# segasai/rvspecfit

Measured on AMD Instinct MI355X. Metric: spectra/sec (CCF+chi2 grid) DESI 3-arm, higher is better.
Workload: dtype f64

## Files before the change

### include/rvsgpu.h

```cpp
#ifndef RVSGPU_H
#define RVSGPU_H
#include <stdint.h>

#ifdef __cplusplus
extern "C" {
#endif

#define RVS_E_ARG (-1)
#define RVS_E_LAUNCH (-2)

#define RVS_ST_SPLINE_RANGE 0x1
#define RVS_ST_SPLINE_GRID 0x2
#define RVS_ST_NONFINITE 0x4
#define RVS_ST_CHOL_FALLBACK 0x8
#define RVS_ST_OUTSIDE_NAN 0x10
#define RVS_ST_CCF_FAILED 0x20
#define RVS_ST_ALLMASKED 0x40
#define RVS_ST_QUAD_ASSERT 0x80
#define RVS_ST_ILLCOND 0x100
#define RVS_ST_NONPOS_MEDIAN 0x200
#define RVS_ST_RBF_NOTPD 0x400

#define RVS_ABI_VERSION 18
int rvs_abi_version(void);
// ... 314 lines not shown
                     int32_t *status, void *stream);

int rvs_ccf_preprocess(const double *lam, const double *spec,
                       const double *espec, const uint8_t *badmask, int npix,
                       int B, int continuum, const double *Eb, const int32_t *El,
                       const double *Cinv, const int32_t *istart, int nnode,
                       const int32_t *bin_start, const int32_t *xind,
                       const double *rw, int nfft, double maxerr,
                       double *proc_spec, double *proc_ivar, double *sse,
                       double *cont, double *pfit, int32_t *status,
                       void *stream);
int rvs_ccf_preprocess_g(const double *lam, const double *spec, const double *espec,
                         const uint8_t *badmask, int npix, int B, int continuum,
                         const double *Eb, const int32_t *El, const double *Cinv,
                         const int32_t *istart, int nnode,
                         const int32_t *bin_start, const int32_t *xind,
                         const double *rw, int nfft, double maxerr,
                         double *proc_spec, double *proc_ivar, double *sse,
                         double *cont, double *pfit, int32_t *status,
                         const int32_t *grid_id, const int32_t *npix_g,
                         const int32_t *nnode_g, void *stream);

int rvs_ccf_fft_pos(int nfft, int f);
int rvs_ccf_xcorr(const double *proc_spec, const double *proc_ivar, int nfft,
                  int B, const double *tfft, const double *tfft2, int T,
                  const double *twid, int continuum, const int32_t *lag_pos,
                  const double *lag_vel, int nlag, const int32_t *ilo,
                  const double *vgrid, int nvel, double beta,
                  const uint8_t *prune, double *chisq, double *work,
                  void *stream);

#define RVS_CCF_MODEL_MAX_NTP 9216
int rvs_ccf_model_rows(const float *dats, int64_t ngrid, const int64_t *sel,
                       int exp_flag, int ntp, int M, double *rows, void *stream);
int rvs_ccf_models_build(const double *rows, const uint8_t *f32row,
                         const double *erows, int ntp, int M, int continuum,
                         const double *Eb, const int32_t *El, const double *Cinv,
                         const int32_t *istart, int nnode, const int32_t *bin_start,
                         const double *lnlam, const double *logl, const int32_t *ihi,
                         int npoints, const double *twid, double *model, double *fft,
                         double *fft2, double *cont, double *pfit, int32_t *status,
                         void *stream);

int rvs_ccf_select(const double *chisq, const double *sse, int narm_sse, int B,
                   int T, const double *vgrid, int nvel, double *res,
                   double *best_ccf, int32_t *status, void *stream);

int rvs_template_nn(const double *params, int B, int ndim, uint32_t log_mask,
                    const double *M, const double *S, int nlayer,
                    const float *const *W, const float *const *b,
                    const int32_t *dims, float *act0, float *act1,
                    double *templ, void *stream);

int rvs_template_nn_grad(const double *params, int B, int ndim, uint32_t log_mask,
                         const double *M, const double *S, int nlayer,
                         const float *const *W, const float *const *b,
                         const int32_t *dims, float *act0, float *act1,
                         double *templ , void *stream);

int rvs_nn_outside(const double *params, int B, int ndim, uint32_t log_mask,
                   const double *M, const double *S, int mapped,
                   const double *xeqs, int nfx, const double *yeqs, int nfy,
                   double *outside, void *stream);

int rvs_nm_begin(int S, int N, double xatol, double fatol, int maxiter,
                 const double *sim, const double *fsim, const int32_t *nit,
                 int32_t *flags, int32_t *list1, double *X1, int32_t *counts,
                 int jbound, void *stream);
int rvs_nm_decide(int N, const double *sim, const double *fsim,
// ... 293 lines not shown
```

### rvspecfit_amd/_lib.py

```python
import ctypes
import os

import torch

_HERE = os.path.dirname(os.path.abspath(__file__))
LIB_PATH = os.path.join(_HERE, 'librvsgpu.so')

P = ctypes.c_void_p
I = ctypes.c_int
L = ctypes.c_int64
D = ctypes.c_double
U = ctypes.c_uint32

SIGNATURES = {
    'rvs_abi_version': (I, []),
    'rvs_option_set': (I, [ctypes.c_char_p, I]),
    'rvs_option_get': (I, [ctypes.c_char_p, P]),
    'rvs_template_polylinear': (I, [P, L, I, P, P, P, I, P, P, U, I, P, I, P, P,
                                    P, P, P]),
    'rvs_template_polylinear_grad': (I, [P, L, I, P, P, P, I, P, P, U, I, P, I, P,
                                         P, P, P, P]),
    'rvs_template_tri': (I, [P, I, P, P, P, I, I, U, I, P, I, P, P, P, P, P]),
    'rvs_template_tri_buckets': (I, [P, I, P, P, P, I, I, U, I, P, P, I, P, P, P,
                                     P, P]),
# ... 91 lines not shown
    'rvs_objective_work_size': (L, [I, I]),
    'rvs_objective_fused': (I, [P, I, I, P, P, P, I, P, D, I, P, P, P, P]),
    'rvs_objective_from_template': (I, [P, I, I, P, P, P, P, I, P, D, I, P, P, P,
                                        P]),
    'rvs_objective_fused_n': (I, [P, I, I, P, P, P, I, P, P, D, I, P, P, P, P]),
    'rvs_objective_from_template_n': (I, [P, I, I, P, P, P, P, I, P, P, D, I, P,
                                          P, P, P]),
    'rvs_objective_grad_ok': (I, [I, I, I, I, I]),
    'rvs_objective_grad_work_size': (L, [I, I, I]),
    'rvs_objective_grad': (I, [P, I, I, I, P, P, P, I, P, D, P, P, P, P, P, P]),
    'rvs_bfgs_run_grad_fused': (I, [P, P, P, P, P, P, I, P, P]),
    'rvs_grid_moments': (I, [P, P, L, P, I, I, I, I, P, P, P, P]),
    'rvs_basis_build': (I, [P, P, I, I, I, I, P, P, P, P, P]),
    'rvs_ccf_tables_build': (I, [P, P, I, I, P, I, I, P, P, P, I, P, P, P, P, P, P,
                                 P]),
    'rvs_ccf_preprocess': (I, [P, P, P, P, I, I, I, P, P, P, P, I, P, P, P, I, D,
                               P, P, P, P, P, P, P]),
    'rvs_ccf_preprocess_g': (I, [P, P, P, P, I, I, I, P, P, P, P, I, P, P, P, I,
                                 D, P, P, P, P, P, P, P, P, P, P]),
    'rvs_ccf_fft_pos': (I, [I, I]),
    'rvs_ccf_xcorr': (I, [P, P, I, I, P, P, I, P, I, P, P, I, P, P, I, D, P, P,
                          P, P]),
    'rvs_ccf_select': (I, [P, P, I, I, I, P, I, P, P, P, P]),
    'rvs_ccf_model_rows': (I, [P, L, P, I, I, I, P, P]),
    'rvs_ccf_models_build': (I, [P, P, P, I, I, I, P, P, P, P, I, P, P, P, P, I, P,
                                 P, P, P, P, P, P, P]),
    'rvs_template_nn': (I, [P, I, I, U, P, P, I, P, P, P, P, P, P, P]),
    'rvs_template_nn_grad': (I, [P, I, I, U, P, P, I, P, P, P, P, P, P, P]),
    'rvs_template_nn_arms': (I, [P, I, I, I, P, P]),
    'rvs_template_nn_arms_n': (I, [P, I, P, I, I, P, P]),
    'rvs_nn_outside': (I, [P, I, I, U, P, P, I, P, I, P, I, P, P]),
    'rvs_rebin_weights': (I, [P, I, P, P, P, P, I, I, P, P]),
    'rvs_rebin_apply': (I, [P, I, L, I, I, P, P, I, P, P, P, I, I, P, P]),
    'rvs_template_normalize': (I, [P, I, I, P, I, D, D, I, I, P, P, P, P]),
    'rvs_rbf_work_size': (L, [I, I]),
    'rvs_rbf_factor': (I, [P, I, I, D, P, P, P, P]),
    'rvs_rbf_solve': (I, [P, I, L, I, I, P, P, P]),
    'rvs_rbf_eval': (I, [P, I, P, I, I, D, P, I, I, P, L, P]),
    'rvs_nn_train_work_size': (L, [I, I, I, P]),
    'rvs_nn_train_grad': (I, [P, P, I, P, I, I, P, P, P, P, P, D, P, P, P, P, P, P]),
    'rvs_nn_adam_step': (I, [I, P, P, P, P, P, P, P, P, P, D, I, P]),
    'rvs_nn_train_epoch': (I, [P, P, I, P, I, I, I, P, P, P, P, P, P, P, P, P, D, D, I,
                               P, P, P, P]),
}

_lib = None
# ... 216 lines not shown
```

### rvspecfit_amd/csrc/ccf.hip

```cpp
#include "common.h"

#define PP_NT 512
#define PP_LOG2NT 9
#define PP_NW (PP_NT / 64)


#define SEL_NB PP_NT
struct SelShared {
  unsigned long long kmin, kmax, result, next, cand[64];
  int hist[SEL_NB];
  int wtot[PP_NW];
  int cnt, nnan, nc, bucket, kk, nle;
};
__device__ __forceinline__ unsigned long long sel_key(double x) {
  const unsigned long long b = (unsigned long long)__double_as_longlong(x);
  return (b >> 63) ? ~b : (b | 0x8000000000000000ull);
}
__device__ __forceinline__ double sel_value(unsigned long long k) {
  const unsigned long long b = (k >> 63) ? (k & 0x7fffffffffffffffull) : ~k;
  return __longlong_as_double((long long)b);
}
__device__ __forceinline__ unsigned long long shfl_xor_u64(unsigned long long v,
                                                           int o) {
  const int lo = __shfl_xor((int)(v & 0xffffffffu), o, 64);
// ... 1020 lines not shown
    return RVS_E_ARG;
  if ((fft != nullptr) != (fft2 != nullptr)) return RVS_E_ARG;
  if (fft) {
    if (npoints < 64 || npoints > 16384 || (npoints & (npoints - 1)) || !twid)
      return RVS_E_ARG;
  }
  const size_t shm = sizeof(double) * 2 * (size_t)ntp;
  static bool attr_set = false;
  if (!attr_set) {
    (void)hipFuncSetAttribute(
        (const void *)ccf_model_kernel, hipFuncAttributeMaxDynamicSharedMemorySize,
        (int)(CCF_MODEL_LDS - sizeof(LMSharedModel) - sizeof(SelShared)));
    (void)hipGetLastError();
    attr_set = true;
  }
  hipLaunchKernelGGL(ccf_model_kernel, dim3(M), dim3(PP_NT), shm, rvs_stream(stream),
                     rows, f32row, erows, ntp, continuum, Eb, El, Cinv, istart, nnode,
                     bin_start, lnlam, logl, ihi, npoints, model, cont, pfit, status);
  RVS_LAUNCH_CHECK();
  if (fft) return ccf_model_rfft(model, npoints, M, twid, fft, fft2, rvs_stream(stream));
  return 0;
}

__device__ __forceinline__ bool nan_less(double a, long long ka, double b,
                                         long long kb) {
  const bool an = !(a == a), bn = !(b == b);
  if (an != bn) return an;
  if (an) return ka < kb;
  return (a < b) || (a == b && ka < kb);
}

__global__ void __launch_bounds__(256)
    ccf_select_kernel(const double *__restrict__ chisq,
                      const double *__restrict__ sse, int narm, int T,
                      const double *__restrict__ vgrid, int nvel,
                      double *__restrict__ res, double *__restrict__ best_ccf,
                      int32_t *__restrict__ status) {
  __shared__ double sv[4];
  __shared__ long long sk[4];
  const int b = blockIdx.x, tid = threadIdx.x;
  double tot = 0;
  for (int a = 0; a < narm; a++) tot += sse[(int64_t)a * gridDim.x + b];
  const double *c = chisq + (int64_t)b * T * nvel;
  double bv = __builtin_inf();
  long long bk = (1ll << 62);
  for (int e = tid; e < T * nvel; e += 256) {
    const double x = c[e] + tot;
    if (nan_less(x, e, bv, bk)) {
      bv = x;
      bk = e;
    }
  }
#pragma unroll
  for (int o = 32; o > 0; o >>= 1) {
// ... 64 lines not shown
```

### rvspecfit_amd/csrc/ccf_fft.hip

```cpp
#include "common.h"

#define XC_NT 512
#define XC_NTW(n2) ((n2) >> 3)

struct XcLds {
  int t1;
  int c0;
  int t1c;
  int ca;
  int lt;
  size_t bytes;
};
#define XW_NT1C 73
#define XW_NLT 256
#define XC_LDS_MAX (159 * 1024)
__host__ __device__ constexpr XcLds xc_lds_pair(int n2, int nlag) {
  const int t1 = n2, c0 = t1 + XC_NTW(n2);
  return {t1, c0, 0, 0, 0,
          sizeof(double2) * (size_t)c0 + sizeof(double) * 2 * (size_t)nlag};
}
__host__ __device__ constexpr XcLds xc_lds_ws(int n2, int nlag, bool ratio) {
  const int t1 = 2 * n2, c0 = t1 + XC_NTW(n2), t1c = c0 + ((nlag + 1) >> 1),
            ca = t1c + XW_NT1C, lt = ca + (ratio ? (nlag + 1) >> 1 : 0);
  return {t1, c0, t1c, ca, lt,
          sizeof(double2) * (size_t)lt + sizeof(int32_t) * (size_t)XW_NLT};
}
__host__ __device__ constexpr XcLds xc_lds_ws2(int n2, int nlag) {
  const int t1 = 4 * n2, c0 = t1 + XC_NTW(n2);
  return {t1, c0, 0, 0, 0,
          sizeof(double2) * (size_t)c0 + sizeof(double) * 2 * (size_t)nlag};
}
__host__ __device__ constexpr bool xc_lds_fits(const XcLds &L, int n2, int nimg,
                                               int nrow, int nlag, bool ws, bool ratio) {
  const size_t D2 = sizeof(double2), D = sizeof(double);
  size_t end = D2 * (size_t)nimg * n2;
  if (D2 * L.t1 < end) return false;
  end = D2 * (L.t1 + XC_NTW(n2));
  if (D2 * L.c0 < end) return false;
  end = D2 * L.c0 + D * (size_t)nrow * nlag;
  if (ws) {
    if (D2 * L.t1c < end) return false;
    end = D2 * (L.t1c + 72);
    if (D2 * L.ca < end) return false;
    end = D2 * L.ca + (ratio ? D * (size_t)nlag : 0);
    if (D2 * L.lt < end) return false;
    end = D2 * L.lt + sizeof(int32_t) * (size_t)XW_NLT;
  }
  return end <= L.bytes && L.bytes <= XC_LDS_MAX;
}
constexpr bool xc_lds_check() {
  for (int nlag = 2; nlag <= 512; nlag++)
    for (int n2 = 2048; n2 <= 4096; n2 *= 2) {
      for (int ratio = 0; ratio < 2; ratio++)
        if (!xc_lds_fits(xc_lds_ws(n2, nlag, ratio), n2, 2, 1, nlag, true, ratio))
          return false;
      if (n2 == 2048 && !xc_lds_fits(xc_lds_ws2(n2, nlag), n2, 4, 2, nlag, false, false))
        return false;
      if (!xc_lds_fits(xc_lds_pair(n2, nlag), n2, 1, 2, nlag, false, false))
        return false;
    }
  return true;
}
static_assert(xc_lds_check(), "an LDS array of a cross-correlation kernel overlaps "
                              "its neighbour or ends beyond the launch's request");

__device__ __forceinline__ double2 cmul(double2 a, double2 b) {
  return make_double2(a.x * b.x - a.y * b.y, a.x * b.y + a.y * b.x);
}
__device__ __forceinline__ double2 cadd(double2 a, double2 b) {
// ... 578 lines not shown
  double2 v[8];
#pragma unroll
  for (int j = 0; j < 8; j++) v[j] = a[base + Mp * j];
  dft8<SIGN>(v);
  if (Mp > 1) {
    double2 w1 = Tc ? Tc[r] : T1[r << (tws - 1)];
    if (SIGN < 0) w1.y = -w1.y;
    v[1] = cmul(v[1], w1);
    const double2 w2 = cmul(w1, w1);
    v[2] = cmul(v[2], w2);
    double2 wc = cmul(w2, w1);
    v[3] = cmul(v[3], wc);
    const double2 w4 = cmul(w2, w2);
    v[4] = cmul(v[4], w4);
    v[7] = cmul(v[7], cmul(w4, wc));
    wc = cmul(w4, w1);
    v[5] = cmul(v[5], wc);
    v[6] = cmul(v[6], cmul(w4, w2));
  }
#pragma unroll
  for (int q = 0; q < 8; q++) a[base + Mp * q] = v[q];
}

template <int LOG2N, bool RATIO>
__global__ void __launch_bounds__(XW_NT)
    ccf_xcorr_ws_kernel(const double2 *__restrict__ work,
                        const double2 *__restrict__ tfft,
                        const double2 *__restrict__ tfft2, int T,
                        const double2 *__restrict__ tw,
                        const int32_t *__restrict__ lag_pos,
                        const double *__restrict__ lag_vel, int nlag,
                        const int32_t *__restrict__ ilo,
                        const double *__restrict__ vgrid, int nvel, double beta,
                        const uint8_t *__restrict__ prune,
                        double *__restrict__ chisq) {
  extern __shared__ double2 fa[];
  constexpr int log2n = LOG2N, n2 = 1 << LOG2N, nfft = 2 * n2, npair = n2 / 2;
  constexpr int NPP = npair / XW_HALF;
  constexpr bool P12 = (LOG2N == 12);
  static_assert(LOG2N == 12 || LOG2N == 11, "plans 8,8,8,8 and 8,8,8,4 only");
  auto img = [&](int i) -> double2 * { return fa + (i & 1) * n2; };
  const XcLds lds = xc_lds_ws(n2, nlag, RATIO);
  const double2 *T1 = fa + lds.t1;
  double *c0 = reinterpret_cast<double *>(fa + lds.c0);
  double2 *T1c = fa + lds.t1c;
  double *cA = reinterpret_cast<double *>(fa + lds.ca);
  int32_t *lt = reinterpret_cast<int32_t *>(fa + lds.lt);
  const int TI = RATIO ? 2 * T : T;
  const int b = blockIdx.x, tid = threadIdx.x;
  const bool producer = tid >= XW_HALF;
  const int pt = tid & (XW_HALF - 1);
  const double inv_n = 1.0 / nfft;
  if (P12 && tid < 72)
    T1c[tid] = tid < 64 ? tw[2 * (tid << 3)] : tw[2 * ((tid - 64) << (log2n - 6))];
  xc_fill_twiddles<XW_NT>(fa + n2, n2, tw);
  XcMasks pmask = {0u, 0u, 0u};
  bool bad = !P12;
  if (P12 && !producer) {
    pmask = xc_load_masks<XW_HALF>(prune, n2);
    const int pos8 = pt & 7;
    const unsigned m = pmask.g;
    bad = m != 0 && !((pos8 == 0 && m == 0x01u) || (pos8 == 7 && m == 0x80u));
  }
  if (P12 && tid < XW_NLT) lt[tid] = -1;
  const bool fold = !__syncthreads_or(bad);
  if (P12) {
    if (fold && tid < nlag) {
      const int p = lag_pos[tid], e = (p >> 1) & 63;
      if (e == 0 || e == 63) lt[(((p >> 7) & 63) << 2) + (e ? 2 : 0) + (p & 1)] = tid;
    }
    __syncthreads();
  }
  const double2 *Sc = work + ((int64_t)b * 2) * (n2 + 1);
  const double2 *Vc = Sc + (n2 + 1);
  typedef int v4i_t __attribute__((ext_vector_type(4)));
  auto ld = [](const __amdgpu_buffer_rsrc_t &r, int off) {
    const v4i_t v = __builtin_amdgcn_raw_buffer_load_b128(r, off, 0, 0);
    return make_double2(__hiloint2double(v.y, v.x), __hiloint2double(v.w, v.z));
  };
  const int nbytes = (n2 + 1) * 16;
  if (producer) {
    double2 Sk[NPP], Vk[NPP], Sm[NPP], Vm[NPP];
#pragma unroll
    for (int u = 0; u < NPP; u++) {
      const int k = 1 + pt + u * XW_HALF, m = n2 - k;
      Sk[u] = Sc[k], Vk[u] = Vc[k], Sm[u] = Sc[m], Vm[u] = Vc[m];
    }
    const __amdgpu_buffer_rsrc_t rT = __builtin_amdgcn_make_buffer_rsrc(
        (void *)tw, 0, (npair + 1) * 16, 0x00020000);
    double2 op[2][5];
    auto issue = [&](int t, int u, double2 *o) {
      const int tt = RATIO ? (t >> 1) : t;
      const __amdgpu_buffer_rsrc_t rF = __builtin_amdgcn_make_buffer_rsrc(
          (void *)(((RATIO && (t & 1)) ? tfft2 : tfft) + (int64_t)tt * (n2 + 1)), 0,
          nbytes, 0x00020000);
      const __amdgpu_buffer_rsrc_t rF2 = __builtin_amdgcn_make_buffer_rsrc(
          (void *)(tfft2 + (int64_t)tt * (n2 + 1)), 0, nbytes, 0x00020000);
      int ptv = pt;
      asm volatile("" : "+v"(ptv));
      const int k = 1 + ptv + u * XW_HALF;
      const int ok = k * 16, om = (n2 - k) * 16;
      if (RATIO) {
        o[0] = ld(rF, ok);
        o[2] = ld(rF, om);
      } else {
        o[0] = ld(rF, ok), o[1] = ld(rF2, ok);
        o[2] = ld(rF, om), o[3] = ld(rF2, om);
      }
      o[4] = ld(rT, ok);
// ... 3 lines not shown
      int ptv = pt;
      asm volatile("" : "+v"(ptv));
      const int k = 1 + ptv + u * XW_HALF, m = n2 - k;
      double2 Xk, Xm;
      if (RATIO) {
        const bool second = (tcur & 1) != 0;
        Xk = cmul(o[0], second ? Vk[u] : Sk[u]);
        Xm = cmul(o[2], second ? Vm[u] : Sm[u]);
      } else {
        const double2 p1 = cmul(o[0], Sk[u]), p2 = cmul(o[1], Vk[u]);
        Xk = make_double2(p2.x - 2 * p1.x, p2.y - 2 * p1.y);
        const double2 q1 = cmul(o[2], Sm[u]), q2 = cmul(o[3], Vm[u]);
        Xm = make_double2(q2.x - 2 * q1.x, q2.y - 2 * q1.y);
      }
      const double2 e = make_double2(Xk.x + Xm.x, Xk.y - Xm.y);
      const double2 d = make_double2(Xk.x - Xm.x, Xk.y + Xm.y);
      const double2 q = cmul(o[4], d);
      dst[k] = make_double2(e.x - q.y, e.y + q.x);
      if (m != k) dst[m] = make_double2(e.x + q.y, -e.y + q.x);
      if (u == NPP - 1 && ptv == 0) {
        double xk, xm;
        if (RATIO) {
          const bool second = (tcur & 1) != 0;
          xk = cmul(second ? dc[1] : dc[0], second ? Vc[0] : Sc[0]).x;
          xm = cmul(second ? dc[3] : dc[2], second ? Vc[n2] : Sc[n2]).x;
        } else {
          const double2 a1 = cmul(dc[0], Sc[0]), a2 = cmul(dc[1], Vc[0]);
          const double2 b1 = cmul(dc[2], Sc[n2]), b2 = cmul(dc[3], Vc[n2]);
          xk = a2.x - 2 * a1.x, xm = b2.x - 2 * b1.x;
        }
        dst[0] = make_double2(xk + xm, xk - xm);
      }
    };
    const bool two = P12 && fold;
    const int nbar = two ? 2 : 5;
    issue(0, 0, op[0]);
    if (NPP == 2) issue(0, 1, op[1]);
    for (int it = -1; it < TI; it++) {
      const int tn = it + 1;
      if (tn < TI) {
        double2 *dst = img(tn);
        {
          const int tt = RATIO ? (tn >> 1) : tn;
          const double2 *Fp = tfft + (int64_t)tt * (n2 + 1);
          const double2 *F2p = tfft2 + (int64_t)tt * (n2 + 1);
          dc[0] = Fp[0], dc[1] = F2p[0], dc[2] = Fp[n2], dc[3] = F2p[n2];
        }
        if (NPP == 2) {
#pragma unroll
          for (int u = 0; u < 2; u++) {
            form(dst, u, op[u], tn);
            if (tn + 1 < TI) issue(tn + 1, u, op[u]);
            __syncthreads();
          }
        } else {
#pragma unroll
          for (int u = 0; u < NPP; u++) {
            if (u + 1 < NPP)
              issue(tn, u + 1, op[(u + 1) & 1]);
            else if (tn + 1 < TI)
              issue(tn + 1, 0, op[(u + 1) & 1]);
            form(dst, u, op[u & 1], tn);
            if (!two || (u & 1)) __syncthreads();
          }
        }
        for (int q = two ? NPP / 2 : NPP; q < nbar; q++) __syncthreads();
      } else {
        for (int q = 0; q < nbar; q++) __syncthreads();
      }
    }
    return;
  }
  const int tvx = min(pt, nvel - 1);
  const int pre_pos = lag_pos[min(pt, nlag - 1)];
  const int pre_lo = ilo[tvx];
  const double pre_xg = vgrid[tvx];
  const double pre_x0 = lag_vel[pre_lo], pre_x1 = lag_vel[pre_lo + 1];
  typedef int v4i32_t __attribute__((ext_vector_type(4)));
  v4i32_t lag = {-1, -1, -1, -1};
  if (P12) lag = reinterpret_cast<const v4i32_t *>(lt)[pt >> 3];
  for (int it = -1; it < TI; it++) {
    if (it < 0) {
      const int nbar = (P12 && fold) ? 2 : 5;
      for (int q = 0; q < nbar; q++) __syncthreads();
      continue;
    }
    double2 *a = img(it);
    double *out = chisq + ((int64_t)b * T + (RATIO ? (it >> 1) : it)) * nvel;
    double pre_old = 0;
    if (beta != 0.0) pre_old = out[tvx];
    if (pt < (n2 >> 3)) xw_pass<1, LOG2N>(a, T1, 0, pt);
    __syncthreads();
    if (pt < (n2 >> 3)) xw_pass<1, LOG2N>(a, T1, 1, pt, P12 ? T1c : nullptr);
    if (P12 && fold) {
      __builtin_amdgcn_fence(__ATOMIC_RELEASE, "wavefront");
      __builtin_amdgcn_wave_barrier();
      __builtin_amdgcn_fence(__ATOMIC_ACQUIRE, "wavefront");
      const int s = pt & 7;
      const int B = pt >> 3;
      const unsigned m0 = pmask.b0 & 1u, m63 = pmask.b7 >> 7;
      if (m0 | m63) {
        double2 v[8];
#pragma unroll
// ... 78 lines not shown
  #pragma unroll
            for (int q = 0; q < 8; q++)
              if (mask & (1u << q)) a[base + q] = v[q];
          }
        }
        __syncthreads();
      }
      if (RATIO) {
        if (pt < nlag) {
          const double c = reinterpret_cast<const double *>(a)[pre_pos] * inv_n;
          if (it & 1)
            c0[pt] = -cA[pt] * cA[pt] / c;
          else
            cA[pt] = c;
        }
      } else if (pt < nlag) {
        c0[pt] = reinterpret_cast<const double *>(a)[pre_pos] * inv_n;
      }
      __syncthreads();
    }
    if ((!RATIO || (it & 1)) && pt < nvel) {
      const double sl = (c0[pre_lo + 1] - c0[pre_lo]) / (pre_x1 - pre_x0);
      const double val = sl * (pre_xg - pre_x0) + c0[pre_lo];
      out[pt] = (beta != 0.0) ? beta * pre_old + val : val;
    }
  }
}

__global__ void __launch_bounds__(XW_NT)
    ccf_xcorr_ws2_kernel(const double2 *__restrict__ work,
                         const double2 *__restrict__ tfft,
                         const double2 *__restrict__ tfft2, int T,
                         const double2 *__restrict__ tw,
                         const int32_t *__restrict__ lag_pos,
                         const double *__restrict__ lag_vel, int nlag,
                         const int32_t *__restrict__ ilo,
                         const double *__restrict__ vgrid, int nvel, double beta,
                         double *__restrict__ chisq) {
  extern __shared__ double2 fa[];
  constexpr int LOG2N = 11, n2 = 1 << LOG2N, nfft = 2 * n2, npair = n2 / 2;
  constexpr int NBAR = 5;
  auto img = [&](int i, int j) -> double2 * { return fa + (((i & 1) << 1) + j) * n2; };
  const XcLds lds = xc_lds_ws2(n2, nlag);
  const double2 *T1 = fa + lds.t1;
  double *c0 = reinterpret_cast<double *>(fa + lds.c0);
  const int b = blockIdx.x, tid = threadIdx.x;
  const bool producer = tid >= XW_HALF;
// ... 108 lines not shown
      dft4<1>(v0, v1, v2, v3);
      a[base] = v0, a[base + 1] = v1, a[base + 2] = v2, a[base + 3] = v3;
    }
    __syncthreads();
    if (pt < nlag) {
      c0[pt] = reinterpret_cast<const double *>(img(it, 0))[pre_pos[0]] * inv_n;
      c0[nlag + pt] = reinterpret_cast<const double *>(img(it, 1))[pre_pos[0]] * inv_n;
    }
    __syncthreads();
    if (pt < nvel) {
      const double dx = pre_x1 - pre_x0, xg = pre_xg - pre_x0;
      const double sl0 = (c0[pre_lo + 1] - c0[pre_lo]) / dx;
      const double val0 = sl0 * xg + c0[pre_lo];
      out0[pt] = (beta != 0.0) ? beta * old0 + val0 : val0;
      if (two) {
        const double sl1 = (c0[nlag + pre_lo + 1] - c0[nlag + pre_lo]) / dx;
        const double val1 = sl1 * xg + c0[nlag + pre_lo];
        out1[pt] = (beta != 0.0) ? beta * old1 + val1 : val1;
      }
    }
  }
}

extern "C" int rvs_ccf_xcorr(const double *proc_spec, const double *proc_ivar,
                             int nfft, int B, const double *tfft,
                             const double *tfft2, int T, const double *twid_,
                             int continuum, const int32_t *lag_pos,
                             const double *lag_vel, int nlag, const int32_t *ilo,
                             const double *vgrid, int nvel, double beta,
                             const uint8_t *prune, double *chisq, double *work,
                             void *stream) {
  int log2n = 0;
  while ((2 << log2n) < nfft) log2n++;
  if ((2 << log2n) != nfft || nfft < 64 || nfft > 16384) return RVS_E_ARG;
  if (B < 1 || T < 1 || T > 65535 || nlag < 2 || nvel < 1) return RVS_E_ARG;
  const int n2 = nfft >> 1;
  const size_t shm1 = xc_lds_pair(n2, 0).bytes;
  const size_t shm2 = xc_lds_pair(n2, nlag).bytes;
  if (shm2 > XC_LDS_MAX) return RVS_E_ARG;
  hipStream_t st = rvs_stream(stream);
  const double2 *tw = reinterpret_cast<const double2 *>(twid_);
  static bool attr_set = false;
  if (!attr_set) {
    (void)hipFuncSetAttribute((const void *)ccf_rfft_kernel<false>,
                              hipFuncAttributeMaxDynamicSharedMemorySize,
                              XC_LDS_MAX);
    (void)hipFuncSetAttribute((const void *)ccf_xcorr_kernel,
                              hipFuncAttributeMaxDynamicSharedMemorySize,
                              XC_LDS_MAX);
    (void)hipGetLastError();
    attr_set = true;
  }
  hipLaunchKernelGGL(ccf_rfft_kernel<false>, dim3(B, 2), dim3(XC_NT), shm1, st,
                     proc_spec, proc_ivar, nfft, log2n, tw,
                     reinterpret_cast<double2 *>(work), (double2 *)nullptr);
  RVS_LAUNCH_CHECK();
  const int G = xc_group(T, nfft);
  {
    const bool ws_on = rvs_opt(RVS_OPT_XC_WS) != 0;
    const bool p12 = (nfft == 8192 && prune), p11 = (nfft == 4096);
    if (ws_on && (p12 || p11) && nlag <= XW_HALF && nvel <= XW_HALF && T >= 2) {
      static bool ws_attr = false;
      if (!ws_attr) {
        (void)hipFuncSetAttribute((const void *)ccf_xcorr_ws_kernel<12, false>,
                                  hipFuncAttributeMaxDynamicSharedMemorySize,
                                  XC_LDS_MAX);
        (void)hipFuncSetAttribute((const void *)ccf_xcorr_ws_kernel<12, true>,
                                  hipFuncAttributeMaxDynamicSharedMemorySize,
                                  XC_LDS_MAX);
        (void)hipFuncSetAttribute((const void *)ccf_xcorr_ws_kernel<11, true>,
                                  hipFuncAttributeMaxDynamicSharedMemorySize,
                                  XC_LDS_MAX);
        (void)hipFuncSetAttribute((const void *)ccf_xcorr_ws2_kernel,
                                  hipFuncAttributeMaxDynamicSharedMemorySize,
                                  XC_LDS_MAX);
        (void)hipGetLastError();
        ws_attr = true;
      }
      const size_t shmw = xc_lds_ws(n2, nlag, !continuum).bytes;
#define RVS_XW_ARGS                                                                 \
  reinterpret_cast<const double2 *>(work), reinterpret_cast<const double2 *>(tfft),  \
      reinterpret_cast<const double2 *>(tfft2), T, tw, lag_pos, lag_vel, nlag, ilo,  \
      vgrid, nvel, beta, prune, chisq
      if (!continuum) {
        if (p12)
          hipLaunchKernelGGL((ccf_xcorr_ws_kernel<12, true>), dim3(B), dim3(XW_NT), shmw,
                             st, RVS_XW_ARGS);
        else
          hipLaunchKernelGGL((ccf_xcorr_ws_kernel<11, true>), dim3(B), dim3(XW_NT), shmw,
                             st, RVS_XW_ARGS);
        RVS_LAUNCH_CHECK();
        return 0;
      }
      if (p12)
        hipLaunchKernelGGL((ccf_xcorr_ws_kernel<12, false>), dim3(B), dim3(XW_NT), shmw, st,
                           reinterpret_cast<const double2 *>(work),
                           reinterpret_cast<const double2 *>(tfft),
                           reinterpret_cast<const double2 *>(tfft2), T, tw, lag_pos,
                           lag_vel, nlag, ilo, vgrid, nvel, beta, prune, chisq);
      else
        hipLaunchKernelGGL(ccf_xcorr_ws2_kernel, dim3(B), dim3(XW_NT),
                           xc_lds_ws2(n2, nlag).bytes, st,
                           reinterpret_cast<const double2 *>(work),
                           reinterpret_cast<const double2 *>(tfft),
                           reinterpret_cast<const double2 *>(tfft2), T, tw, lag_pos,
                           lag_vel, nlag, ilo, vgrid, nvel, beta, chisq);
      RVS_LAUNCH_CHECK();
      return 0;
    }
  }
  const int bmax = G ? (int)(0x7fffffffll / xc_nblocks(T, 1, G)) : 65535;
  for (int b0 = 0; b0 < B; b0 += bmax) {
    const int nb = (B - b0 < bmax) ? (B - b0) : bmax;
    const dim3 grid = G ? dim3((unsigned)xc_nblocks(T, nb, G)) : dim3(T, nb);
    hipLaunchKernelGGL(
        ccf_xcorr_kernel, grid, dim3(XB_NT), shm2, st,
        reinterpret_cast<const double2 *>(work) + (int64_t)b0 * 2 * (n2 + 1),
        nfft, log2n, reinterpret_cast<const double2 *>(tfft),
        reinterpret_cast<const double2 *>(tfft2), T, tw, continuum, lag_pos,
        lag_vel, nlag, ilo, vgrid, nvel, beta, prune,
        chisq + (int64_t)b0 * T * nvel, nb, G);
    RVS_LAUNCH_CHECK();
  }
  return 0;
}
```

### rvspecfit_amd/csrc/common.h

```cpp
#pragma once
#include <hip/hip_runtime.h>
#include <stdint.h>
#include "../../include/rvsgpu.h"
#include "options.h"

#define RVS_C_KMS 299792.458

#define RVS_LAUNCH_CHECK()                         \
  do {                                             \
    if (hipGetLastError() != hipSuccess) return RVS_E_LAUNCH; \
  } while (0)

static inline hipStream_t rvs_stream(void *s) { return (hipStream_t)s; }

__device__ __forceinline__ double wave_sum(double v) {
#pragma unroll
  for (int o = 32; o > 0; o >>= 1) v += __shfl_xor(v, o, 64);
  return v;
}
template <int CTRL, int ROW_MASK, int BANK_MASK>
__device__ __forceinline__ double dpp_get(double v) {
  const int lo = __double2loint(v), hi = __double2hiint(v);
  const int lo2 =
      __builtin_amdgcn_update_dpp(0, lo, CTRL, ROW_MASK, BANK_MASK, false);
  const int hi2 =
      __builtin_amdgcn_update_dpp(0, hi, CTRL, ROW_MASK, BANK_MASK, false);
  return __hiloint2double(hi2, lo2);
}

__device__ __forceinline__ double wave_sum_to63(double v) {
  double t = v + dpp_get<0x111, 0xf, 0xf>(v);
  t += dpp_get<0x112, 0xf, 0xf>(v);
  t += dpp_get<0x113, 0xf, 0xf>(v);
  t += dpp_get<0x114, 0xf, 0xe>(t);
  t += dpp_get<0x118, 0xf, 0xc>(t);
  t += dpp_get<0x142, 0xa, 0xf>(t);
  t += dpp_get<0x143, 0xc, 0xf>(t);
  return t;
}

__device__ __forceinline__ int wave_sum_i(int v) {
#pragma unroll
  for (int o = 32; o > 0; o >>= 1) v += __shfl_xor(v, o, 64);
  return v;
}
__device__ __forceinline__ double wave_max(double v) {
#pragma unroll
  for (int o = 32; o > 0; o >>= 1) v = fmax(v, __shfl_xor(v, o, 64));
  return v;
}

template <int NW>
__device__ __forceinline__ double block_sum(double v, double *red) {
  v = wave_sum(v);
  const int w = threadIdx.x >> 6;
  __syncthreads();
  if ((threadIdx.x & 63) == 0) red[w] = v;
  __syncthreads();
  double t = 0;
#pragma unroll
  for (int i = 0; i < NW; i++) t += red[i];
// ... 32 lines not shown
```

### rvspecfit_amd/engine.py

```python
import ctypes
import threading

import numpy as np
import torch

from . import _lib
from . import ccf_tables

SPEED_OF_LIGHT = 299792.458

KTIMERS = None


class _ktime:

    def __init__(self, name, units=1):
        self.name, self.units = name, units

    def __enter__(self):
        if KTIMERS is not None:
            self.e0 = torch.cuda.Event(enable_timing=True)
            self.e0.record()

    def __exit__(self, *a):
# ... 1359 lines not shown
        if cc['T'] != Tn:
            raise RuntimeError('CCF template counts are inconsistent across setups')
        if (not np.array_equal(ref['params'], cc['params'])
                or not np.array_equal(ref['vsinis'], cc['vsinis'],
                                      equal_nan=True)):
            raise RuntimeError('The parameters of the CCF templates do not match')
    tabs = [a.ccf_tables(libs[a.name], config) for a in batch.arms]
    nvel = len(tabs[0]['vgrid_host'])
    pre = [ccf_preprocess(a, libs[a.name], config) for a in batch.arms]
    sse = torch.stack([p['sse'] for p in pre]).contiguous()
    status = torch.zeros(S, dtype=torch.int32, device=dev)
    for p in pre:
        status |= p['status']
    if max_chunk is None:
        max_chunk = max(1, min(S, int(2e9 // (Tn * nvel * 8))))
        nchunk = -(-S // max_chunk)
        max_chunk = -(-S // nchunk)
    res = torch.empty((S, 4), dtype=torch.float64, device=dev)
    best_ccf = torch.empty((S, nvel), dtype=torch.float64, device=dev)
    allchi = None
    for a, b in _chunks(S, max_chunk):
        n = b - a
        acc = torch.empty((n, Tn, nvel), dtype=torch.float64, device=dev)
        for ia, arm in enumerate(batch.arms):
            cc = libs[arm.name].ccf_set(config)
            T = tabs[ia]
            nfft = cc['npoints']
            work = torch.empty((n, 2, nfft // 2 + 1, 2), dtype=torch.float64,
                               device=dev)
            with _ktime('ccf_xcorr', n):
              rc = L.rvs_ccf_xcorr(
                _lib.ptr(pre[ia]['proc_spec'][a:b]),
                _lib.ptr(pre[ia]['proc_ivar'][a:b]), nfft, n,
                _lib.ptr(cc['fft']), _lib.ptr(cc['fft2']), Tn,
                _lib.ptr(T['twid']), int(cc['continuum']),
                _lib.ptr(T['lag_pos']), _lib.ptr(T['lag_vel']), T['nlag'],
                _lib.ptr(T['ilo']), _lib.ptr(T['vgrid']), nvel,
                0.0 if ia == 0 else 1.0, _lib.ptr(T['prune']), _lib.ptr(acc),
                _lib.ptr(work), _lib.stream())
            _lib.check(rc, 'rvs_ccf_xcorr')
        sse_c = sse[:, a:b].contiguous()
        rc = L.rvs_ccf_select(_lib.ptr(acc), _lib.ptr(sse_c), len(batch.arms),
                              n, Tn, _lib.ptr(tabs[0]['vgrid']), nvel,
                              _lib.ptr(res[a:b]), _lib.ptr(best_ccf[a:b]),
                              _lib.ptr(status[a:b]), _lib.stream())
        _lib.check(rc, 'rvs_ccf_select')
        if keep_all:
            allchi = acc + sse_c.sum(dim=0)[:, None, None]
    out = dict(best_id=res[:, 0].long(), best_vel=res[:, 1].contiguous(),
               best_pix=res[:, 2].long(), best_ccf=best_ccf, status=status,
               vel_grid=tabs[0]['vgrid'], vel_grid_host=tabs[0]['vgrid_host'],
               proc_spec=[p['proc_spec'] for p in pre],
               proc_ivar=[p['proc_ivar'] for p in pre],
               steps=[t['step'] for t in tabs])
    if keep_all:
        out['all_chisqs'] = allchi
    return out
```

Baseline: 82980.

## Fuse real FFT and best-template selection into the warp-specialized xcorr kernel

For the nfft 8192 pruned path, the warp-specialized cross-correlation kernel now loads proc_spec/proc_ivar, runs the forward FFT passes in LDS and unfolds the real spectrum itself, so the separate rfft kernel and its global work buffer are skipped. On the last arm, a select epilogue tracks the running NaN-aware minimum chi2 per block, then refines velocity by parabolic interpolation and writes res, best_ccf and status, replacing the standalone select kernel. The aim is to cut two kernel launches and the global round-trip of FFT and chisq data. In exchange the kernel does more in-block work and needs extra LDS and barriers, which may change occupancy.

```diff
diff --git a/include/rvsgpu.h b/include/rvsgpu.h
--- a/include/rvsgpu.h
+++ b/include/rvsgpu.h
@@ -360,6 +360,8 @@
                          const int32_t *nnode_g, void *stream);
 
 int rvs_ccf_fft_pos(int nfft, int f);
+int64_t rvs_ccf_xcorr_work_size(int nfft, int B, int T, int nlag, int nvel,
+                                int has_prune);
 int rvs_ccf_xcorr(const double *proc_spec, const double *proc_ivar, int nfft,
                   int B, const double *tfft, const double *tfft2, int T,
                   const double *twid, int continuum, const int32_t *lag_pos,
@@ -383,6 +385,15 @@
 int rvs_ccf_select(const double *chisq, const double *sse, int narm_sse, int B,
                    int T, const double *vgrid, int nvel, double *res,
                    double *best_ccf, int32_t *status, void *stream);
+
+int rvs_ccf_xcorr_select(const double *proc_spec, const double *proc_ivar, int nfft,
+                         int B, const double *tfft, const double *tfft2, int T,
+                         const double *twid, int continuum, const int32_t *lag_pos,
+                         const double *lag_vel, int nlag, const int32_t *ilo,
+                         const double *vgrid, int nvel, double beta,
+                         const uint8_t *prune, double *chisq, double *work,
+                         const double *sse, int narm, double *res, double *best_ccf,
+                         int32_t *status, void *stream);
 
 int rvs_template_nn(const double *params, int B, int ndim, uint32_t log_mask,
                     const double *M, const double *S, int nlayer,
diff --git a/rvspecfit_amd/_lib.py b/rvspecfit_amd/_lib.py
--- a/rvspecfit_amd/_lib.py
+++ b/rvspecfit_amd/_lib.py
@@ -137,6 +137,9 @@
     'rvs_ccf_xcorr': (I, [P, P, I, I, P, P, I, P, I, P, P, I, P, P, I, D, P, P,
                           P, P]),
     'rvs_ccf_select': (I, [P, P, I, I, I, P, I, P, P, P, P]),
+    'rvs_ccf_xcorr_work_size': (L, [I, I, I, I, I, I]),
+    'rvs_ccf_xcorr_select': (I, [P, P, I, I, P, P, I, P, I, P, P, I, P, P, I, D, P, P,
+                                 P, P, I, P, P, P, P]),
     'rvs_ccf_model_rows': (I, [P, L, P, I, I, I, P, P]),
     'rvs_ccf_models_build': (I, [P, P, P, I, I, I, P, P, P, P, I, P, P, P, P, I, P,
                                  P, P, P, P, P, P, P]),
diff --git a/rvspecfit_amd/csrc/ccf.hip b/rvspecfit_amd/csrc/ccf.hip
--- a/rvspecfit_amd/csrc/ccf.hip
+++ b/rvspecfit_amd/csrc/ccf.hip
@@ -1066,14 +1066,6 @@
   return 0;
 }
 
-__device__ __forceinline__ bool nan_less(double a, long long ka, double b,
-                                         long long kb) {
-  const bool an = !(a == a), bn = !(b == b);
-  if (an != bn) return an;
-  if (an) return ka < kb;
-  return (a < b) || (a == b && ka < kb);
-}
-
 __global__ void __launch_bounds__(256)
     ccf_select_kernel(const double *__restrict__ chisq,
                       const double *__restrict__ sse, int narm, int T,
diff --git a/rvspecfit_amd/csrc/ccf_fft.hip b/rvspecfit_amd/csrc/ccf_fft.hip
--- a/rvspecfit_amd/csrc/ccf_fft.hip
+++ b/rvspecfit_amd/csrc/ccf_fft.hip
@@ -9,25 +9,27 @@
   int t1c;
   int ca;
   int lt;
+  int dc;
   size_t bytes;
 };
 #define XW_NT1C 73
 #define XW_NLT 256
+#define XW_NDC 4
 #define XC_LDS_MAX (159 * 1024)
 __host__ __device__ constexpr XcLds xc_lds_pair(int n2, int nlag) {
   const int t1 = n2, c0 = t1 + XC_NTW(n2);
-  return {t1, c0, 0, 0, 0,
+  return {t1, c0, 0, 0, 0, 0,
           sizeof(double2) * (size_t)c0 + sizeof(double) * 2 * (size_t)nlag};
 }
 __host__ __device__ constexpr XcLds xc_lds_ws(int n2, int nlag, bool ratio) {
   const int t1 = 2 * n2, c0 = t1 + XC_NTW(n2), t1c = c0 + ((nlag + 1) >> 1),
-            ca = t1c + XW_NT1C, lt = ca + (ratio ? (nlag + 1) >> 1 : 0);
-  return {t1, c0, t1c, ca, lt,
-          sizeof(double2) * (size_t)lt + sizeof(int32_t) * (size_t)XW_NLT};
+            ca = t1c + XW_NT1C, lt = ca + (ratio ? (nlag + 1) >> 1 : 0),
+            dc = lt + (int)(sizeof(int32_t) * XW_NLT / sizeof(double2));
+  return {t1, c0, t1c, ca, lt, dc, sizeof(double2) * (size_t)(dc + XW_NDC)};
 }
 __host__ __device__ constexpr XcLds xc_lds_ws2(int n2, int nlag) {
   const int t1 = 4 * n2, c0 = t1 + XC_NTW(n2);
-  return {t1, c0, 0, 0, 0,
+  return {t1, c0, 0, 0, 0, 0,
           sizeof(double2) * (size_t)c0 + sizeof(double) * 2 * (size_t)nlag};
 }
 __host__ __device__ constexpr bool xc_lds_fits(const XcLds &L, int n2, int nimg,
@@ -45,6 +47,8 @@
     end = D2 * L.ca + (ratio ? D * (size_t)nlag : 0);
     if (D2 * L.lt < end) return false;
     end = D2 * L.lt + sizeof(int32_t) * (size_t)XW_NLT;
+    if (D2 * L.dc < end) return false;
+    end = D2 * (L.dc + XW_NDC);
   }
   return end <= L.bytes && L.bytes <= XC_LDS_MAX;
 }
@@ -669,9 +673,18 @@
   for (int q = 0; q < 8; q++) a[base + Mp * q] = v[q];
 }
 
-template <int LOG2N, bool RATIO>
+struct XwSelect {
+  const double *sse;
+  int narm;
+  double *res;
+  double *best_ccf;
+  int32_t *status;
+};
+template <int LOG2N, bool RATIO, bool SELECT = false>
 __global__ void __launch_bounds__(XW_NT)
     ccf_xcorr_ws_kernel(const double2 *__restrict__ work,
+                        const double *__restrict__ proc_spec,
+                        const double *__restrict__ proc_ivar,
                         const double2 *__restrict__ tfft,
                         const double2 *__restrict__ tfft2, int T,
                         const double2 *__restrict__ tw,
@@ -680,12 +693,14 @@
                         const int32_t *__restrict__ ilo,
                         const double *__restrict__ vgrid, int nvel, double beta,
                         const uint8_t *__restrict__ prune,
-                        double *__restrict__ chisq) {
+                        double *__restrict__ chisq, const XwSelect sel) {
   extern __shared__ double2 fa[];
   constexpr int log2n = LOG2N, n2 = 1 << LOG2N, nfft = 2 * n2, npair = n2 / 2;
   constexpr int NPP = npair / XW_HALF;
   constexpr bool P12 = (LOG2N == 12);
+  constexpr int NBAR_SEL = 2;
   static_assert(LOG2N == 12 || LOG2N == 11, "plans 8,8,8,8 and 8,8,8,4 only");
+  static_assert(!SELECT || P12, "the select epilogue belongs to the nfft 8192 form");
   auto img = [&](int i) -> double2 * { return fa + (i & 1) * n2; };
   const XcLds lds = xc_lds_ws(n2, nlag, RATIO);
   const double2 *T1 = fa + lds.t1;
@@ -693,6 +708,7 @@
   double2 *T1c = fa + lds.t1c;
   double *cA = reinterpret_cast<double *>(fa + lds.ca);
   int32_t *lt = reinterpret_cast<int32_t *>(fa + lds.lt);
+  double2 *dcs = fa + lds.dc;
   const int TI = RATIO ? 2 * T : T;
   const int b = blockIdx.x, tid = threadIdx.x;
   const bool producer = tid >= XW_HALF;
@@ -701,6 +717,18 @@
   if (P12 && tid < 72)
     T1c[tid] = tid < 64 ? tw[2 * (tid << 3)] : tw[2 * ((tid - 64) << (log2n - 6))];
   xc_fill_twiddles<XW_NT>(fa + n2, n2, tw);
+  if constexpr (P12) {
+    const double *ps = proc_spec + (int64_t)b * nfft;
+    const double *pi = proc_ivar + (int64_t)b * nfft;
+#pragma unroll
+    for (int j = 0; j < n2 / XW_NT; j++) {
+      const int n = tid + j * XW_NT;
+      const double s0 = ps[2 * n], s1 = ps[2 * n + 1];
+      const double i0 = pi[2 * n], i1 = pi[2 * n + 1];
+      fa[n] = make_double2(s0 * i0, s1 * i1);
+      fa[n2 + n] = make_double2(i0, i1);
+    }
+  }
   XcMasks pmask = {0u, 0u, 0u};
   bool bad = !P12;
   if (P12 && !producer) {
@@ -718,8 +746,20 @@
     }
     __syncthreads();
   }
-  const double2 *Sc = work + ((int64_t)b * 2) * (n2 + 1);
-  const double2 *Vc = Sc + (n2 + 1);
+  if constexpr (P12) {
+    double2 *ap = fa + (producer ? n2 : 0);
+#pragma unroll
+    for (int p = 0; p < 4; p++) {
+      xw_pass<-1, LOG2N>(ap, T1, p, pt);
+      __syncthreads();
+    }
+  }
+  const double2 *Sc = P12 ? nullptr : work + ((int64_t)b * 2) * (n2 + 1);
+  const double2 *Vc = P12 ? nullptr : Sc + (n2 + 1);
+  auto spec_dc = [&](int i) -> double2 {
+    if constexpr (P12) return dcs[i];
+    return ((i & 2) ? Vc : Sc)[(i & 1) ? n2 : 0];
+  };
   typedef int v4i_t __attribute__((ext_vector_type(4)));
   auto ld = [](const __amdgpu_buffer_rsrc_t &r, int off) {
     const v4i_t v = __builtin_amdgcn_raw_buffer_load_b128(r, off, 0, 0);
@@ -728,10 +768,35 @@
   const int nbytes = (n2 + 1) * 16;
   if (producer) {
     double2 Sk[NPP], Vk[NPP], Sm[NPP], Vm[NPP];
-#pragma unroll
-    for (int u = 0; u < NPP; u++) {
-      const int k = 1 + pt + u * XW_HALF, m = n2 - k;
-      Sk[u] = Sc[k], Vk[u] = Vc[k], Sm[u] = Sc[m], Vm[u] = Vc[m];
+    if constexpr (P12) {
+      auto unfold = [](double2 zk, double2 zm, double2 w) {
+        const double2 e = make_double2(zk.x + zm.x, zk.y - zm.y);
+        const double2 d = make_double2(zk.x - zm.x, zk.y + zm.y);
+        const double2 q = cmul(w, d);
+        return make_double2(0.5 * (e.x + q.y), -(0.5 * (e.y - q.x)));
+      };
+      const double2 *Z0 = fa, *Z1 = fa + n2;
+#pragma unroll
+      for (int u = 0; u < NPP; u++) {
+        const int k = 1 + pt + u * XW_HALF, m = n2 - k;
+        const int pk = fft_pos(k, log2n), pm = fft_pos(m, log2n);
+        const double2 wk = twid<-1>(tw, k, nfft), wm = twid<-1>(tw, m, nfft);
+        const double2 s_k = Z0[pk], s_m = Z0[pm], v_k = Z1[pk], v_m = Z1[pm];
+        Sk[u] = unfold(s_k, s_m, wk), Sm[u] = unfold(s_m, s_k, wm);
+        Vk[u] = unfold(v_k, v_m, wk), Vm[u] = unfold(v_m, v_k, wm);
+      }
+      if (pt == 0) {
+        const double2 s = Z0[0], v = Z1[0];
+        dcs[0] = make_double2(s.x + s.y, -0.0), dcs[1] = make_double2(s.x - s.y, -0.0);
+        dcs[2] = make_double2(v.x + v.y, -0.0), dcs[3] = make_double2(v.x - v.y, -0.0);
+      }
+      __syncthreads();
+    } else {
+#pragma unroll
+      for (int u = 0; u < NPP; u++) {
+        const int k = 1 + pt + u * XW_HALF, m = n2 - k;
+        Sk[u] = Sc[k], Vk[u] = Vc[k], Sm[u] = Sc[m], Vm[u] = Vc[m];
+      }
     }
     const __amdgpu_buffer_rsrc_t rT = __builtin_amdgcn_make_buffer_rsrc(
         (void *)tw, 0, (npair + 1) * 16, 0x00020000);
@@ -781,11 +846,11 @@
         double xk, xm;
         if (RATIO) {
           const bool second = (tcur & 1) != 0;
-          xk = cmul(second ? dc[1] : dc[0], second ? Vc[0] : Sc[0]).x;
-          xm = cmul(second ? dc[3] : dc[2], second ? Vc[n2] : Sc[n2]).x;
+          xk = cmul(second ? dc[1] : dc[0], spec_dc(second ? 2 : 0)).x;
+          xm = cmul(second ? dc[3] : dc[2], spec_dc(second ? 3 : 1)).x;
         } else {
-          const double2 a1 = cmul(dc[0], Sc[0]), a2 = cmul(dc[1], Vc[0]);
-          const double2 b1 = cmul(dc[2], Sc[n2]), b2 = cmul(dc[3], Vc[n2]);
+          const double2 a1 = cmul(dc[0], spec_dc(0)), a2 = cmul(dc[1], spec_dc(2));
+          const double2 b1 = cmul(dc[2], spec_dc(1)), b2 = cmul(dc[3], spec_dc(3));
           xk = a2.x - 2 * a1.x, xm = b2.x - 2 * b1.x;
         }
         dst[0] = make_double2(xk + xm, xk - xm);
@@ -828,6 +893,8 @@
         for (int q = 0; q < nbar; q++) __syncthreads();
       }
     }
+    if constexpr (SELECT)
+      for (int q = 0; q < NBAR_SEL; q++) __syncthreads();
     return;
   }
   const int tvx = min(pt, nvel - 1);
@@ -838,6 +905,11 @@
   typedef int v4i32_t __attribute__((ext_vector_type(4)));
   v4i32_t lag = {-1, -1, -1, -1};
   if (P12) lag = reinterpret_cast<const v4i32_t *>(lt)[pt >> 3];
+  double tot = 0, bv = __builtin_inf();
+  long long bk = (1ll << 62);
+  if constexpr (SELECT)
+    for (int a = 0; a < sel.narm; a++) tot += sel.sse[(int64_t)a * gridDim.x + b];
+  if constexpr (P12) __syncthreads();
   for (int it = -1; it < TI; it++) {
     if (it < 0) {
       const int nbar = (P12 && fold) ? 2 : 5;
@@ -962,7 +1034,57 @@
     if ((!RATIO || (it & 1)) && pt < nvel) {
       const double sl = (c0[pre_lo + 1] - c0[pre_lo]) / (pre_x1 - pre_x0);
       const double val = sl * (pre_xg - pre_x0) + c0[pre_lo];
-      out[pt] = (beta != 0.0) ? beta * pre_old + val : val;
+      const double o = (beta != 0.0) ? beta * pre_old + val : val;
+      out[pt] = o;
+      if constexpr (SELECT) {
+        const double x = o + tot;
+        const long long key = (long long)(RATIO ? (it >> 1) : it) * nvel + pt;
+        if (nan_less(x, key, bv, bk)) bv = x, bk = key;
+      }
+    }
+  }
+  if constexpr (SELECT) {
+    auto block_min = [&](double2 *part, double &v, long long &k) {
+      wave_nan_min(v, k);
+      if ((pt & 63) == 0) part[pt >> 6] = make_double2(v, __longlong_as_double(k));
+      __threadfence_block();
+      __syncthreads();
+      v = part[0].x, k = __double_as_longlong(part[0].y);
+      for (int w = 1; w < XW_HALF / 64; w++) {
+        const double ov = part[w].x;
+        const long long ok = __double_as_longlong(part[w].y);
+        if (nan_less(ov, ok, v, k)) v = ov, k = ok;
+      }
+    };
+    block_min(fa, bv, bk);
+    const int best_id = (int)(bk / nvel);
+    const double *row = chisq + ((int64_t)b * T + best_id) * nvel;
+    double *xs = reinterpret_cast<double *>(fa + 16);
+    double mv = __builtin_inf();
+    long long bp = (1ll << 62);
+    if (pt < nvel) {
+      mv = row[pt] + tot, bp = pt;
+      sel.best_ccf[(int64_t)b * nvel + pt] = mv;
+      xs[pt] = mv;
+    }
+    block_min(fa + 8, mv, bp);
+    if (pt == 0) {
+      double vel = vgrid[bp];
+      if (bp != 0 && bp != nvel - 1) {
+        const double xa = vgrid[bp - 1], xb = vgrid[bp], xc = vgrid[bp + 1];
+        const double ya = xs[bp - 1], yb = xs[bp], yc = xs[bp + 1];
+        const double d1 = (yb - ya) / (xb - xa), d2 = (yc - yb) / (xc - xb);
+        const double a2 = (d2 - d1) / (xc - xa);
+        if (a2 > 0) vel = xb - (d1 + a2 * (xb - xa)) / (2 * a2);
+      }
+      int st = 0;
+      if (!(fabs(mv) <= 1.79e308)) st |= RVS_ST_CCF_FAILED;
+      double *r = sel.res + (int64_t)b * 4;
+      r[0] = best_id;
+      r[1] = vel;
+      r[2] = bp;
+      r[3] = mv;
+      if (st && sel.status) atomicOr(&sel.status[b], st);
     }
   }
 }
@@ -1117,14 +1239,24 @@
   }
 }
 
-extern "C" int rvs_ccf_xcorr(const double *proc_spec, const double *proc_ivar,
-                             int nfft, int B, const double *tfft,
-                             const double *tfft2, int T, const double *twid_,
-                             int continuum, const int32_t *lag_pos,
-                             const double *lag_vel, int nlag, const int32_t *ilo,
-                             const double *vgrid, int nvel, double beta,
-                             const uint8_t *prune, double *chisq, double *work,
-                             void *stream) {
+static bool xc_takes_ws12(int nfft, int T, int nlag, int nvel, bool has_prune) {
+  return rvs_opt(RVS_OPT_XC_WS) != 0 && nfft == 8192 && has_prune && nlag <= XW_HALF &&
+         nvel <= XW_HALF && T >= 2;
+}
+extern "C" int64_t rvs_ccf_xcorr_work_size(int nfft, int B, int T, int nlag, int nvel,
+                                           int has_prune) {
+  if (nfft < 64 || B < 1) return RVS_E_ARG;
+  return xc_takes_ws12(nfft, T, nlag, nvel, has_prune != 0)
+             ? 0
+             : (int64_t)B * 2 * ((nfft >> 1) + 1) * 2;
+}
+
+static int xc_launch(const double *proc_spec, const double *proc_ivar, int nfft, int B,
+                     const double *tfft, const double *tfft2, int T, const double *twid_,
+                     int continuum, const int32_t *lag_pos, const double *lag_vel,
+                     int nlag, const int32_t *ilo, const double *vgrid, int nvel,
+                     double beta, const uint8_t *prune, double *chisq, double *work,
+                     void *stream, const XwSelect *psel) {
   int log2n = 0;
   while ((2 << log2n) < nfft) log2n++;
   if ((2 << log2n) != nfft || nfft < 64 || nfft > 16384) return RVS_E_ARG;
@@ -1146,21 +1278,32 @@
     (void)hipGetLastError();
     attr_set = true;
   }
-  hipLaunchKernelGGL(ccf_rfft_kernel<false>, dim3(B, 2), dim3(XC_NT), shm1, st,
-                     proc_spec, proc_ivar, nfft, log2n, tw,
-                     reinterpret_cast<double2 *>(work), (double2 *)nullptr);
-  RVS_LAUNCH_CHECK();
+  const bool ws_on = rvs_opt(RVS_OPT_XC_WS) != 0;
+  const bool p12 = (nfft == 8192 && prune), p11 = (nfft == 4096);
+  const bool ws = ws_on && (p12 || p11) && nlag <= XW_HALF && nvel <= XW_HALF && T >= 2;
+  if (psel && !xc_takes_ws12(nfft, T, nlag, nvel, prune != nullptr)) return RVS_E_ARG;
+  const XwSelect sel = psel ? *psel : XwSelect{nullptr, 0, nullptr, nullptr, nullptr};
+  if (!(ws && p12)) {
+    hipLaunchKernelGGL(ccf_rfft_kernel<false>, dim3(B, 2), dim3(XC_NT), shm1, st,
+                       proc_spec, proc_ivar, nfft, log2n, tw,
+                       reinterpret_cast<double2 *>(work), (double2 *)nullptr);
+    RVS_LAUNCH_CHECK();
+  }
   const int G = xc_group(T, nfft);
   {
-    const bool ws_on = rvs_opt(RVS_OPT_XC_WS) != 0;
-    const bool p12 = (nfft == 8192 && prune), p11 = (nfft == 4096);
-    if (ws_on && (p12 || p11) && nlag <= XW_HALF && nvel <= XW_HALF && T >= 2) {
+    if (ws) {
       static bool ws_attr = false;
       if (!ws_attr) {
         (void)hipFuncSetAttribute((const void *)ccf_xcorr_ws_kernel<12, false>,
                                   hipFuncAttributeMaxDynamicSharedMemorySize,
                                   XC_LDS_MAX);
         (void)hipFuncSetAttribute((const void *)ccf_xcorr_ws_kernel<12, true>,
+                                  hipFuncAttributeMaxDynamicSharedMemorySize,
+                                  XC_LDS_MAX);
+        (void)hipFuncSetAttribute((const void *)ccf_xcorr_ws_kernel<12, false, true>,
+                                  hipFuncAttributeMaxDynamicSharedMemorySize,
+                                  XC_LDS_MAX);
+        (void)hipFuncSetAttribute((const void *)ccf_xcorr_ws_kernel<12, true, true>,
                                   hipFuncAttributeMaxDynamicSharedMemorySize,
                                   XC_LDS_MAX);
         (void)hipFuncSetAttribute((const void *)ccf_xcorr_ws_kernel<11, true>,
@@ -1174,9 +1317,19 @@
       }
       const size_t shmw = xc_lds_ws(n2, nlag, !continuum).bytes;
 #define RVS_XW_ARGS                                                                 \
-  reinterpret_cast<const double2 *>(work), reinterpret_cast<const double2 *>(tfft),  \
-      reinterpret_cast<const double2 *>(tfft2), T, tw, lag_pos, lag_vel, nlag, ilo,  \
-      vgrid, nvel, beta, prune, chisq
+  reinterpret_cast<const double2 *>(work), proc_spec, proc_ivar,                     \
+      reinterpret_cast<const double2 *>(tfft), reinterpret_cast<const double2 *>(tfft2), \
+      T, tw, lag_pos, lag_vel, nlag, ilo, vgrid, nvel, beta, prune, chisq, sel
+      if (psel) {
+        if (!continuum)
+          hipLaunchKernelGGL((ccf_xcorr_ws_kernel<12, true, true>), dim3(B), dim3(XW_NT),
+                             shmw, st, RVS_XW_ARGS);
+        else
+          hipLaunchKernelGGL((ccf_xcorr_ws_kernel<12, false, true>), dim3(B), dim3(XW_NT),
+                             shmw, st, RVS_XW_ARGS);
+        RVS_LAUNCH_CHECK();
+        return 0;
+      }
       if (!continuum) {
         if (p12)
           hipLaunchKernelGGL((ccf_xcorr_ws_kernel<12, true>), dim3(B), dim3(XW_NT), shmw,
@@ -1189,10 +1342,7 @@
       }
       if (p12)
         hipLaunchKernelGGL((ccf_xcorr_ws_kernel<12, false>), dim3(B), dim3(XW_NT), shmw, st,
-                           reinterpret_cast<const double2 *>(work),
-                           reinterpret_cast<const double2 *>(tfft),
-                           reinterpret_cast<const double2 *>(tfft2), T, tw, lag_pos,
-                           lag_vel, nlag, ilo, vgrid, nvel, beta, prune, chisq);
+                           RVS_XW_ARGS);
       else
         hipLaunchKernelGGL(ccf_xcorr_ws2_kernel, dim3(B), dim3(XW_NT),
                            xc_lds_ws2(n2, nlag).bytes, st,
@@ -1219,3 +1369,32 @@
   }
   return 0;
 }
+
+extern "C" int rvs_ccf_xcorr(const double *proc_spec, const double *proc_ivar,
+                             int nfft, int B, const double *tfft,
+                             const double *tfft2, int T, const double *twid_,
+                             int continuum, const int32_t *lag_pos,
+                             const double *lag_vel, int nlag, const int32_t *ilo,
+                             const double *vgrid, int nvel, double beta,
+                             const uint8_t *prune, double *chisq, double *work,
+                             void *stream) {
+  return xc_launch(proc_spec, proc_ivar, nfft, B, tfft, tfft2, T, twid_, continuum,
+                   lag_pos, lag_vel, nlag, ilo, vgrid, nvel, beta, prune, chisq, work,
+                   stream, nullptr);
+}
+
+extern "C" int rvs_ccf_xcorr_select(const double *proc_spec, const double *proc_ivar,
+                                    int nfft, int B, const double *tfft,
+                                    const double *tfft2, int T, const double *twid_,
+                                    int continuum, const int32_t *lag_pos,
+                                    const double *lag_vel, int nlag, const int32_t *ilo,
+                                    const double *vgrid, int nvel, double beta,
+                                    const uint8_t *prune, double *chisq, double *work,
+                                    const double *sse, int narm, double *res,
+                                    double *best_ccf, int32_t *status, void *stream) {
+  if (!sse || narm < 0 || !res || !best_ccf) return RVS_E_ARG;
+  const XwSelect sel = {sse, narm, res, best_ccf, status};
+  return xc_launch(proc_spec, proc_ivar, nfft, B, tfft, tfft2, T, twid_, continuum,
+                   lag_pos, lag_vel, nlag, ilo, vgrid, nvel, beta, prune, chisq, work,
+                   stream, &sel);
+}
diff --git a/rvspecfit_amd/csrc/common.h b/rvspecfit_amd/csrc/common.h
--- a/rvspecfit_amd/csrc/common.h
+++ b/rvspecfit_amd/csrc/common.h
@@ -37,6 +37,25 @@
   t += dpp_get<0x142, 0xa, 0xf>(t);
   t += dpp_get<0x143, 0xc, 0xf>(t);
   return t;
+}
+
+__device__ __forceinline__ bool nan_less(double a, long long ka, double b,
+                                         long long kb) {
+  const bool an = !(a == a), bn = !(b == b);
+  if (an != bn) return an;
+  if (an) return ka < kb;
+  return (a < b) || (a == b && ka < kb);
+}
+__device__ __forceinline__ void wave_nan_min(double &v, long long &k) {
+#pragma unroll
+  for (int o = 32; o > 0; o >>= 1) {
+    const double ov = __shfl_xor(v, o, 64);
+    const long long ok = __shfl_xor(k, o, 64);
+    if (nan_less(ov, ok, v, k)) {
+      v = ov;
+      k = ok;
+    }
+  }
 }
 
 __device__ __forceinline__ int wave_sum_i(int v) {
diff --git a/rvspecfit_amd/engine.py b/rvspecfit_amd/engine.py
--- a/rvspecfit_amd/engine.py
+++ b/rvspecfit_amd/engine.py
@@ -1405,29 +1405,40 @@
     for a, b in _chunks(S, max_chunk):
         n = b - a
         acc = torch.empty((n, Tn, nvel), dtype=torch.float64, device=dev)
+        sse_c = sse[:, a:b].contiguous()
+        selected = False
         for ia, arm in enumerate(batch.arms):
             cc = libs[arm.name].ccf_set(config)
             T = tabs[ia]
             nfft = cc['npoints']
-            work = torch.empty((n, 2, nfft // 2 + 1, 2), dtype=torch.float64,
-                               device=dev)
+            nwork = L.rvs_ccf_xcorr_work_size(nfft, n, Tn, T['nlag'], nvel,
+                                              int(T['prune'] is not None))
+            work = (torch.empty(nwork, dtype=torch.float64, device=dev)
+                    if nwork > 0 else None)
+            args = (_lib.ptr(pre[ia]['proc_spec'][a:b]),
+                    _lib.ptr(pre[ia]['proc_ivar'][a:b]), nfft, n,
+                    _lib.ptr(cc['fft']), _lib.ptr(cc['fft2']), Tn,
+                    _lib.ptr(T['twid']), int(cc['continuum']),
+                    _lib.ptr(T['lag_pos']), _lib.ptr(T['lag_vel']), T['nlag'],
+                    _lib.ptr(T['ilo']), _lib.ptr(T['vgrid']), nvel,
+                    0.0 if ia == 0 else 1.0, _lib.ptr(T['prune']), _lib.ptr(acc),
+                    _lib.ptr(work))
             with _ktime('ccf_xcorr', n):
-              rc = L.rvs_ccf_xcorr(
-                _lib.ptr(pre[ia]['proc_spec'][a:b]),
-                _lib.ptr(pre[ia]['proc_ivar'][a:b]), nfft, n,
-                _lib.ptr(cc['fft']), _lib.ptr(cc['fft2']), Tn,
-                _lib.ptr(T['twid']), int(cc['continuum']),
-                _lib.ptr(T['lag_pos']), _lib.ptr(T['lag_vel']), T['nlag'],
-                _lib.ptr(T['ilo']), _lib.ptr(T['vgrid']), nvel,
-                0.0 if ia == 0 else 1.0, _lib.ptr(T['prune']), _lib.ptr(acc),
-                _lib.ptr(work), _lib.stream())
+              rc = -1
+              if ia == len(batch.arms) - 1:
+                  rc = L.rvs_ccf_xcorr_select(
+                      *args, _lib.ptr(sse_c), len(batch.arms), _lib.ptr(res[a:b]),
+                      _lib.ptr(best_ccf[a:b]), _lib.ptr(status[a:b]), _lib.stream())
+                  selected = rc == 0
+              if rc != 0:
+                  rc = L.rvs_ccf_xcorr(*args, _lib.stream())
             _lib.check(rc, 'rvs_ccf_xcorr')
-        sse_c = sse[:, a:b].contiguous()
-        rc = L.rvs_ccf_select(_lib.ptr(acc), _lib.ptr(sse_c), len(batch.arms),
-                              n, Tn, _lib.ptr(tabs[0]['vgrid']), nvel,
-                              _lib.ptr(res[a:b]), _lib.ptr(best_ccf[a:b]),
-                              _lib.ptr(status[a:b]), _lib.stream())
-        _lib.check(rc, 'rvs_ccf_select')
+        if not selected:
+            rc = L.rvs_ccf_select(_lib.ptr(acc), _lib.ptr(sse_c), len(batch.arms),
+                                  n, Tn, _lib.ptr(tabs[0]['vgrid']), nvel,
+                                  _lib.ptr(res[a:b]), _lib.ptr(best_ccf[a:b]),
+                                  _lib.ptr(status[a:b]), _lib.stream())
+            _lib.check(rc, 'rvs_ccf_select')
         if keep_all:
             allchi = acc + sse_c.sum(dim=0)[:, None, None]
     out = dict(best_id=res[:, 0].long(), best_vel=res[:, 1].contiguous(),
```

Measured after the change: 84690, median of 6. 1.02x the previous value.
